# thangktran/HardwareAwareOptimalQuantumCircuitCuttingAndKnitting

Measured on AMD Instinct MI355X. Metric: subcircuit-instances/s (full-knit wall time = ms_per_step), syc 32 p=2, higher is better.
Workload: dtype f64

## Files before the change

### hardwareawareoptimalquantumcircuitcuttingandknitting_amd/_lib.py

```python
from __future__ import annotations

import ctypes
import os
import threading

_HERE = os.path.dirname(os.path.abspath(__file__))
LIB_PATH = os.environ.get("QKNIT_LIB") or os.path.join(_HERE, "libqknit.so")

c_i32, c_i64, c_u32, c_u64 = ctypes.c_int32, ctypes.c_int64, ctypes.c_uint32, ctypes.c_uint64
c_vp, c_dp, c_lp = ctypes.c_void_p, ctypes.POINTER(ctypes.c_double), ctypes.POINTER(ctypes.c_int64)


class QkPass(ctypes.Structure):
    _fields_ = [("tile_mask", c_u64), ("group_begin", c_i32), ("group_end", c_i32),
                ("flags", c_i32), ("traced_local", c_u32)]


class QkProgram(ctypes.Structure):
    _fields_ = [("n", c_i32), ("n_eff", c_i32), ("m", c_i32), ("n_slots", c_i32),
                ("packed", c_i32), ("n_passes", c_i32), ("passes", ctypes.POINTER(QkPass)),
                ("ops", c_vp), ("groups", c_vp), ("mats", c_vp)]


class QkLowrankPlan(ctypes.Structure):
# ... 54 lines not shown
    "qk_rank_factors": (c_i32, [c_vp, c_i64, c_vp, c_vp, ctypes.c_double, ctypes.c_double, ctypes.c_double,
                                ctypes.c_int, c_vp, c_vp, c_vp]),
    "qk_prep_workspace_bytes": (c_i32, [c_vp, c_i64, c_i64, ctypes.POINTER(c_i64)]),
    "qk_prep_operands": (c_i32, [c_vp, ctypes.c_int, ctypes.c_int, c_vp, c_vp, c_i64, c_i64, c_vp, ctypes.c_int,
                                 c_vp, c_vp, c_i64, c_i64, c_vp, c_vp, c_vp, c_vp, c_vp, c_vp, c_i64]),
    "qk_compress_operands": (c_i32, [c_vp, ctypes.c_int, ctypes.c_int, c_vp, c_vp, c_i64, c_vp, c_vp, c_vp, c_i64,
                                     c_vp]),
    "qk_compress_operands_ld": (c_i32, [c_vp, ctypes.c_int, ctypes.c_int, c_vp, c_vp, c_i64, c_i64, c_vp, c_i64, c_vp,
                                        c_vp, c_i64, c_i64, c_vp, c_i64]),
    "qk_compress_probe_v": (c_i32, [c_vp, ctypes.c_int, ctypes.c_int, c_vp, c_vp, c_i64, c_i64, c_vp, c_i64, c_vp, c_vp,
                                    c_i64, c_i64, c_vp, c_i64, c_vp, c_i64, c_vp, c_i64]),
    "qk_probe_errors_vpart": (c_i32, [c_vp, ctypes.c_int, ctypes.c_int, c_vp, c_i64, c_i64, c_vp, c_i64, c_vp, c_vp,
                                      c_i64, c_vp, c_vp, ctypes.c_double, ctypes.c_double, c_vp, c_vp, c_vp, c_i64,
                                      c_vp]),
    "qk_probe_workspace_bytes": (c_i32, [c_vp, c_i64, ctypes.POINTER(c_i64)]),
    "qk_probe_errors": (c_i32, [c_vp, ctypes.c_int, ctypes.c_int, c_vp, c_i64, c_i64, c_vp, c_i64, c_vp, c_vp, c_i64,
                                c_i64, c_vp, c_i64, c_vp, c_vp, ctypes.c_double, ctypes.c_double, c_vp, c_vp, c_vp,
                                c_i64]),
    "qk_probe_errors_tally": (c_i32, [c_vp, ctypes.c_int, ctypes.c_int, c_vp, c_i64, c_i64, c_vp, c_i64, c_vp, c_vp, c_i64,
                                c_i64, c_vp, c_i64, c_vp, c_vp, ctypes.c_double, ctypes.c_double, c_vp, c_vp, c_vp,
                                c_i64, c_vp]),
    "qk_probe_accept": (c_i32, [c_vp, c_vp, ctypes.c_int, c_vp, ctypes.c_double, ctypes.c_double, c_vp, c_vp]),
    "qk_rank_tally": (c_i32, [c_vp, c_vp, c_vp, c_vp]),
    "qk_knit_workspace_bytes": (c_i32, [ctypes.POINTER(QkKnitPlan), ctypes.POINTER(c_i64)]),
    "qk_knit": (c_i32, [c_vp, ctypes.POINTER(QkKnitPlan), c_vp, c_vp, c_i64, c_vp]),
    "qk_khatri_rao": (c_i32, [c_vp, c_i64, c_i64, c_i64, c_vp, c_i64, c_vp, c_i64, c_vp]),
    "qk_gather_rows": (c_i32, [c_vp, c_i64, c_i64, c_vp, c_vp, c_vp, c_vp]),
    "qk_npd_workspace_bytes": (c_i32, [c_i64, c_i64, ctypes.POINTER(c_i64)]),
    "qk_threshold_count": (c_i32, [c_vp, c_i64, c_vp, ctypes.c_double, c_vp, c_i64, c_vp]),
    "qk_npd": (c_i32, [c_vp, c_i64, c_vp, ctypes.c_double, c_i64, c_vp, c_i64, c_vp, c_vp, c_vp]),
    "qk_qd_from_rows": (c_i32, [c_vp, c_i64, c_i64, c_vp, c_vp, ctypes.c_double, c_vp]),
    "qk_qd_merge": (c_i32, [c_vp, c_i64, c_vp, c_vp, c_i64, c_vp, c_vp, ctypes.c_double, c_i64, c_vp]),
    "qk_qd_axpby": (c_i32, [c_vp, c_i64, ctypes.c_double, c_vp, ctypes.c_double, c_vp, ctypes.c_double, c_vp]),
    "qk_hellinger": (c_i32, [c_vp, c_i64, c_vp, c_vp, c_vp]),
    "qk_knit_lowrank_workspace_bytes": (c_i32, [c_vp, c_vp, ctypes.POINTER(c_i64)]),
    "qk_knit_lowrank": (c_i32, [c_vp, c_vp, c_vp, c_vp, c_vp, c_i64, c_vp, c_vp]),
    "qk_comm_unique_id": (c_i32, [c_vp]),
    "qk_comm_init": (c_i32, [c_vp, c_vp, ctypes.c_int, ctypes.c_int, ctypes.POINTER(c_vp)]),
    "qk_comm_destroy": (c_i32, [c_vp]),
    "qk_comm_size": (c_i32, [c_vp, ctypes.POINTER(ctypes.c_int), ctypes.POINTER(ctypes.c_int)]),
    "qk_allreduce": (c_i32, [c_vp, c_vp, c_vp, c_vp, c_i64]),
    "qk_reduce": (c_i32, [c_vp, c_vp, c_vp, c_vp, c_i64, ctypes.c_int]),
    "qk_allgather": (c_i32, [c_vp, c_vp, c_vp, c_vp, c_i64]),
    "qk_alltoall": (c_i32, [c_vp, c_vp, c_vp, c_vp, c_i64]),
    "qk_knit_select_workspace_bytes": (c_i32, [ctypes.c_int, c_u64, c_u64, ctypes.POINTER(c_i64)]),
    "qk_knit_select": (c_i32, [c_vp, ctypes.c_int, c_i64, c_vp, c_i64, c_vp, c_i64, c_u64, c_u64, ctypes.c_double,
# ... 58 lines not shown
```

### hardwareawareoptimalquantumcircuitcuttingandknitting_amd/csrc/internal.h

```cpp
#ifndef QKNIT_INTERNAL_H
#define QKNIT_INTERNAL_H

#include <hip/hip_runtime.h>

#include <string>

#include "../../include/qknit.h"

struct qk_ctx {
    int device;
    hipStream_t own;
    hipStream_t stream;
    int cus;
    std::string err;
};

size_t npd_pairs_bytes(int64_t count);
int npd_pairs_bits(qk_ctx* ctx, int64_t count, const int64_t* keys, const double* vals, int key_bits, void* ws,
                   int64_t ws_bytes, int64_t* out_keys, double* out_vals, int64_t* n_out_dev);

#endif
```

### hardwareawareoptimalquantumcircuitcuttingandknitting_amd/csrc/qknit.hip

```cpp
#include <hip/hip_runtime.h>

#include <cstdlib>

#include <cstdint>
#include <cstdio>
#include <cstring>
#include <string>

#include "internal.h"
#include "sweep_ops.h"

namespace {

constexpr int TILE = 1 << QK_TILE_BITS;
constexpr int NT = 256;

int fail(qk_ctx* ctx, int code, const char* fmt, const char* detail = "") {
    if (ctx) {
        char buf[512];
        snprintf(buf, sizeof(buf), fmt, detail);
        ctx->err = buf;
    }
    return code;
}
// ... 1348 lines not shown
static int stream_cus(hipStream_t s, int device) {
    int cus = 0;
    if (hipDeviceGetAttribute(&cus, hipDeviceAttributeMultiprocessorCount, device) != hipSuccess || cus < 1)
        cus = 1;
    uint32_t mask[32] = {0};
    if (s && hipExtStreamGetCUMask(s, 32, mask) == hipSuccess) {
        int n = 0;
        for (uint32_t w : mask) n += __builtin_popcount(w);
        if (n > 0 && n < cus) return n;
    }
    return cus;
}

int qk_ctx_create(int device, qk_ctx** out) {
    if (!out) return QK_EARG;
    *out = nullptr;
    if (hipSetDevice(device) != hipSuccess) return QK_EHIP;
    qk_ctx* c = new qk_ctx();
    c->device = device;
    if (hipStreamCreateWithFlags(&c->own, hipStreamNonBlocking) != hipSuccess) {
        delete c;
        return QK_EHIP;
    }
    c->stream = c->own;
    c->cus = stream_cus(c->own, device);
    *out = c;
    return QK_OK;
}

int qk_ctx_destroy(qk_ctx* ctx) {
    if (!ctx) return QK_EARG;
    (void)hipSetDevice(ctx->device);
    (void)hipStreamSynchronize(ctx->own);
    (void)hipStreamDestroy(ctx->own);
    delete ctx;
    return QK_OK;
}

int qk_ctx_set_stream(qk_ctx* ctx, void* s) {
    if (!ctx) return QK_EARG;
    if ((hipStream_t)s != ctx->stream || s == nullptr) ctx->cus = stream_cus((hipStream_t)s, ctx->device);
    ctx->stream = (hipStream_t)s;
    return QK_OK;
}

int qk_stream_create_cu_masked(int device, const uint32_t* cu_mask, int mask_words, void** stream) {
    if (!stream || !cu_mask || mask_words < 1 || mask_words > 32) return QK_EARG;
    *stream = nullptr;
    if (hipSetDevice(device) != hipSuccess) return QK_EHIP;
    int n = 0;
    for (int w = 0; w < mask_words; ++w) n += __builtin_popcount(cu_mask[w]);
    if (n == 0) return QK_EARG;
    hipStream_t s = nullptr;
    if (hipExtStreamCreateWithCUMask(&s, (uint32_t)mask_words, cu_mask) != hipSuccess) return QK_EHIP;
    *stream = s;
    return QK_OK;
// ... 321 lines not shown
```

### hardwareawareoptimalquantumcircuitcuttingandknitting_amd/csrc/qknit_plan.hip

```cpp
#include <hip/hip_runtime.h>

#include <algorithm>
#include <cstdlib>
#include <string>
#include <vector>

#include "internal.h"

namespace {

int pfail(qk_ctx* ctx, int code, const std::string& msg) {
    if (ctx) ctx->err = msg;
    return code;
}

__global__ void qk_pdep_keys_kernel(int64_t n, uint64_t mask, int64_t* keys) {
    for (int64_t x = blockIdx.x * (int64_t)blockDim.x + threadIdx.x; x < n; x += (int64_t)gridDim.x * blockDim.x) {
        uint64_t m = mask, k = 0, bit = 1;
        for (; m; m &= m - 1, bit <<= 1)
            if ((uint64_t)x & bit) k |= m & (~m + 1);
        keys[x] = (int64_t)k;
    }
}

// ... 242 lines not shown

int qk_knit_lowrank(qk_ctx* ctx, const qk_lowrank_plan* p, const double* q_a, const double* q_b, void* workspace,
                    int64_t workspace_bytes, double* out, int32_t* rank_out) {
    if (!ctx) return QK_EARG;
    LowrankLayout L;
    std::string why;
    int rc = lowrank_layout(ctx, p, L, why);
    if (rc) return pfail(ctx, rc, why);
    if (!q_a || !q_b || !out || !workspace || workspace_bytes < L.total)
        return pfail(ctx, QK_EARG, "qk_knit_lowrank: null rows / output, or workspace below qk_knit_lowrank_workspace_bytes");
    if (hipSetDevice(ctx->device) != hipSuccess) return pfail(ctx, QK_EHIP, "qk_knit_lowrank: hipSetDevice");
    char* ws = static_cast<char*>(workspace);
    auto D = [&](int64_t off) { return reinterpret_cast<double*>(ws + off); };
    const int K = p->terms;
    const int64_t NA = int64_t(1) << __builtin_popcountll(p->mask_a), NB = int64_t(1) << __builtin_popcountll(p->mask_b);
    double *XA = D(L.xa), *XB = D(L.xb), *G = D(L.g), *U = D(L.u);
    int32_t* r = reinterpret_cast<int32_t*>(ws + L.r);
    int32_t* k = reinterpret_cast<int32_t*>(ws + L.k);
    rc = qk_prep_operands(ctx, K, (int)p->rows_a, p->wt_a, q_a, NA, NA, XA, (int)p->rows_b, p->wt_b, q_b, NB, NB, XB,
                          p->probes, G, G + K * K, U, D(L.prep), L.prep_bytes);
    if (!rc) rc = qk_rank_factors(ctx, K, G, G + K * K, p->lam_tol, p->s_tol, p->s_abs, LR_RMAX, D(L.ta), D(L.tb), r);
    if (!rc) rc = qk_compress_operands(ctx, K, LR_RMAX, D(L.ta), XA, NA, D(L.a2), D(L.tb), XB, NB, D(L.b2));
    if (!rc)
        rc = qk_probe_errors(ctx, K, LR_RMAX, XA, NA, NA, D(L.a2), NA, U, D(L.b2), NB, NB, p->probes, NB, D(L.e2), r,
                             p->rank_tol, p->rank_tol_rel, k, D(L.err), D(L.probe), L.probe_bytes);
    if (!rc)
        rc = qk_knit_outer_stream_range(ctx, p->nbits, LR_RMAX, D(L.a2), NA, D(L.b2), NB, p->mask_a, p->mask_b, 0,
                                        int64_t(1) << p->nbits, k, out);
    if (rc) return rc;
    int64_t* ka = L.ka >= 0 ? reinterpret_cast<int64_t*>(ws + L.ka) : nullptr;
    int64_t* kb = L.kb >= 0 ? reinterpret_cast<int64_t*>(ws + L.kb) : nullptr;
    if (ka) hipLaunchKernelGGL(qk_pdep_keys_kernel, dim3(grid_of(NA)), dim3(256), 0, ctx->stream, NA, p->mask_a, ka);
    if (kb) hipLaunchKernelGGL(qk_pdep_keys_kernel, dim3(grid_of(NB)), dim3(256), 0, ctx->stream, NB, p->mask_b, kb);
    const int64_t sa = ka ? 0 : int64_t(1) << __builtin_ctzll(p->mask_a);
    const int64_t sb = kb ? 0 : int64_t(1) << __builtin_ctzll(p->mask_b);
    rc = qk_gemm_keyed_pred(ctx, NA, NB, K, XA, NA, XB, NB, ka, sa, kb, sb, out, 0, k);
    if (rc) return rc;
    if (rank_out) hipLaunchKernelGGL(qk_copy_i32_kernel, dim3(1), dim3(1), 0, ctx->stream, k, rank_out);
    if (hipGetLastError() != hipSuccess) return pfail(ctx, QK_EHIP, "qk_knit_lowrank: launch failed");
    return QK_OK;
}

}
```

### hardwareawareoptimalquantumcircuitcuttingandknitting_amd/csrc/qknit_prep.hip

```cpp
#include <hip/hip_runtime.h>

#include <cstdint>
#include <string>

#include "internal.h"

namespace {

typedef double d4_t __attribute__((ext_vector_type(4)));
typedef double d2_t __attribute__((ext_vector_type(2)));

constexpr int PK = 64;
constexpr int PCT = 128;
constexpr int PNP = 16;
constexpr int PTH = 512;
constexpr int XLD = PCT + 2;
constexpr int PG_BLK = 10;
constexpr int PPG = PG_BLK * 256;
constexpr int PPA = PPG;
constexpr int PPB = PPG + PK * PNP;
__host__ __device__ constexpr int prep_tri(int bi, int bj) { return bi * 4 - bi * (bi - 1) / 2 + (bj - bi); }

struct PrepSide {
    const double* Wt;
// ... 687 lines not shown
}

int fail(qk_ctx* ctx, int code, const char* msg) {
    ctx->err = msg;
    return code;
}

#ifndef QK_PREP_SPLIT
#define QK_PREP_SPLIT 1
#endif
bool prep_split(qk_ctx* ctx, int64_t NA, int64_t NB) {
    const int64_t tiles = (NA > NB ? NA : NB) / PCT;
    const int64_t g = (int64_t)(ctx->cus > 0 ? ctx->cus : 256) * QK_PREP_WG_PER_CU;
    return QK_PREP_SPLIT && tiles > 0 && 2 * tiles <= g;
}

int prep_grid(qk_ctx* ctx, int64_t NA, int64_t NB) {
    const int64_t tiles = (NA > NB ? NA : NB) / PCT;
    if (prep_split(ctx, NA, NB)) return (int)(2 * tiles);
    const int64_t g = (int64_t)(ctx->cus > 0 ? ctx->cus : 256) * QK_PREP_WG_PER_CU;
    return (int)(tiles < g ? (tiles > 0 ? tiles : 1) : g);
}

}

extern "C" {

int qk_prep_workspace_bytes(qk_ctx* ctx, int64_t NA, int64_t NB, int64_t* bytes) {
    if (!ctx || !bytes) return QK_EARG;
    *bytes = (int64_t)prep_grid(ctx, NA, NB) * (PPA + PPB) * (int64_t)sizeof(double);
    return QK_OK;
}

int qk_prep_operands(qk_ctx* ctx, int K, int RA, const double* WtA, const double* qA, int64_t ldqA, int64_t NA,
                     double* XA, int RB, const double* WtB, const double* qB, int64_t ldqB, int64_t NB, double* XB,
                     const double* probes, double* GA, double* GB, double* U, double* work, int64_t work_bytes) {
    if (!ctx) return QK_EARG;
    if (K < 2 || K > PK || (K & 1) || RA < 1 || RB < 1)
        return fail(ctx, QK_EARG, "qk_prep_operands: need even 2 <= K <= 64 and R >= 1 on both sides");
    if (((reinterpret_cast<uintptr_t>(WtA) | reinterpret_cast<uintptr_t>(WtB) | reinterpret_cast<uintptr_t>(qA) |
          reinterpret_cast<uintptr_t>(qB)) & 15) || (ldqA & 1) || (ldqB & 1))
        return fail(ctx, QK_EARG, "qk_prep_operands: 16-B aligned Wt / q and even ldq required");
    if (NA < PCT || NB < PCT || NA % PCT || NB % PCT || ldqA < NA || ldqB < NB)
        return fail(ctx, QK_EARG, "qk_prep_operands: columns must be a positive multiple of 128 (ldq >= N)");
    if (!WtA || !qA || !XA || !WtB || !qB || !XB || !probes || !GA || !GB || !U || !work)
        return fail(ctx, QK_EARG, "qk_prep_operands: null buffer");
// ... 102 lines not shown
    return QK_OK;
}

int qk_probe_workspace_bytes(qk_ctx* ctx, int64_t NA, int64_t* bytes) {
    if (!ctx || !bytes) return QK_EARG;
    *bytes = (int64_t)(PV_GRID * PV_PART + probe_grid_d(ctx, NA) * PE) * (int64_t)sizeof(double);
    return QK_OK;
}

int qk_probe_errors(qk_ctx* ctx, int K, int rmax, const double* XA, int64_t ldx, int64_t NA, const double* A2,
                    int64_t lda2, const double* U, const double* B2, int64_t ldb2, int64_t NB, const double* probes,
                    int64_t ldp, double* e2, const int32_t* r_dev, double tol, double rel_tol, int32_t* k_out,
                    double* err_out, double* work, int64_t work_bytes) {
    return qk_probe_errors_tally(ctx, K, rmax, XA, ldx, NA, A2, lda2, U, B2, ldb2, NB, probes, ldp, e2, r_dev, tol,
                                 rel_tol, k_out, err_out, work, work_bytes, nullptr);
}

int qk_probe_errors_tally(qk_ctx* ctx, int K, int rmax, const double* XA, int64_t ldx, int64_t NA, const double* A2,
                          int64_t lda2, const double* U, const double* B2, int64_t ldb2, int64_t NB,
                          const double* probes, int64_t ldp, double* e2, const int32_t* r_dev, double tol,
                          double rel_tol, int32_t* k_out, double* err_out, double* work, int64_t work_bytes,
                          int64_t* tally) {
    if (!ctx) return QK_EARG;
    if (K < 1 || K > PK || rmax < 1 || rmax > 8 || NA < 16 || NA % 16 || NB < 4 || NB % 4)
        return fail(ctx, QK_EARG, "qk_probe_errors: need 1 <= K <= 64, 1 <= rmax <= 8, NA % 16 == 0, NB % 4 == 0");
    if (!XA || !A2 || !U || !B2 || !probes || !work || (k_out && !r_dev) || (tally && !k_out))
        return fail(ctx, QK_EARG, "qk_probe_errors: null buffer");
    if (ldx < NA || ldb2 < NB || ldp < NB) return fail(ctx, QK_EARG, "qk_probe_errors: leading dimension");
    const int gd = probe_grid_d(ctx, NA);
    if (work_bytes < (int64_t)(PV_GRID * PV_PART + gd * PE) * (int64_t)sizeof(double))
        return fail(ctx, QK_EARG, "qk_probe_errors: workspace too small (qk_probe_workspace_bytes)");
    if (hipSetDevice(ctx->device) != hipSuccess) return fail(ctx, QK_EHIP, "qk_probe_errors: hipSetDevice");
    double* vpart = work;
    double* epart = work + PV_GRID * PV_PART;
    hipLaunchKernelGGL(qk_probe_v_kernel, dim3(PV_GRID), dim3(256), 0, ctx->stream, rmax, B2, ldb2, NB, probes, ldp,
                       vpart);
    hipLaunchKernelGGL(qk_probe_d_kernel, dim3(gd), dim3(256), 0, ctx->stream, K, rmax, XA, ldx, NA, A2, lda2, U, vpart,
                       PV_GRID, epart);
    hipLaunchKernelGGL(qk_probe_accept_kernel, dim3(1), dim3(256), 0, ctx->stream, epart, gd, r_dev, tol, rel_tol, e2,
                       k_out, err_out, tally);
    const hipError_t e = hipGetLastError();
    if (e != hipSuccess) return fail(ctx, QK_EHIP, (std::string("qk_probe_errors: ") + hipGetErrorString(e)).c_str());
    return QK_OK;
}

__global__ __launch_bounds__(64) void qk_rank_tally_kernel(const int32_t* __restrict__ r, const int32_t* __restrict__ k,
                                                          int64_t* __restrict__ acc) {
    if (threadIdx.x == 0) {
        const int rv = *r, kv = *k;
        acc[0] += rv == 0 ? 1 : 0;
        acc[1] += (rv > 0 && kv == 0) ? 1 : 0;
        acc[2] = kv;
        acc[3] += 1;
    }
}

int qk_rank_tally(qk_ctx* ctx, const int32_t* r_dev, const int32_t* k_dev, int64_t* acc) {
    if (!ctx) return QK_EARG;
    if (!r_dev || !k_dev || !acc) return fail(ctx, QK_EARG, "qk_rank_tally: null buffer");
    if (hipSetDevice(ctx->device) != hipSuccess) return fail(ctx, QK_EHIP, "qk_rank_tally: hipSetDevice");
    hipLaunchKernelGGL(qk_rank_tally_kernel, dim3(1), dim3(64), 0, ctx->stream, r_dev, k_dev, acc);
    const hipError_t e = hipGetLastError();
    if (e != hipSuccess) return fail(ctx, QK_EHIP, (std::string("qk_rank_tally: ") + hipGetErrorString(e)).c_str());
    return QK_OK;
}

// ... 14 lines not shown
```

### hardwareawareoptimalquantumcircuitcuttingandknitting_amd/engine.py

```python
from __future__ import annotations

import atexit
import contextlib
import ctypes
import dataclasses
import hashlib
import logging
import os
import threading
from dataclasses import dataclass, field
from time import perf_counter

import numpy as np

from . import _lib
from .fragment_program import (FragmentProgram, JobTable, basis_reduce, build_jobs, compile_fragment,
                               dedup_labels)
from .knit_plan import LabelSpace, deposit_keys, factor_vgate
from .sweep_plan import K_SLOT, EncodedProgram, encode

_torch = None


def torch():
# ... 1440 lines not shown
    ctx.check(ctx.lib.qk_probe_workspace_bytes(ctx.handle, NA, ctypes.byref(need)), "qk_probe_workspace_bytes")
    key = (str(dev), T.cuda.current_stream(dev).cuda_stream)
    work = _PROBE_WORK.get(key)
    if work is None or work.numel() * 8 < need.value:
        work = _PROBE_WORK[key] = T.empty(max(need.value // 8, 1), dtype=T.float64, device=dev)
    e2 = T.empty(2 * N_PROBES, dtype=T.float64, device=dev)
    k = T.empty(1, dtype=T.int32, device=dev) if r is not None else None
    err = T.empty(1, dtype=T.float64, device=dev) if r is not None else None
    assert tally is None or (r is not None and tally.dtype == T.int64 and tally.numel() == 4)
    if vpart is not None:
        assert vpart.is_contiguous() and vpart.shape[1:] == (8, N_PROBES)
        ctx.check(ctx.lib.qk_probe_errors_vpart(ctx.handle, K, rmax, XA.data_ptr(), XA.stride(0), NA,
                                                A2.data_ptr() + 8 * off, A2.shape[1], U.data_ptr(), vpart.data_ptr(),
                                                vpart.shape[0], e2.data_ptr(), _ptr(r), tol, rel_tol, _ptr(k), _ptr(err),
                                                work.data_ptr(), work.numel() * 8, _ptr(tally)), "qk_probe_errors_vpart")
        return e2, k, err
    ctx.check(ctx.lib.qk_probe_errors_tally(ctx.handle, K, rmax, XA.data_ptr(), XA.stride(0), NA, A2.data_ptr() + 8 * off,
                                            A2.shape[1], U.data_ptr(), B2.data_ptr(), NB, NB, probes.data_ptr(), NB,
                                            e2.data_ptr(), _ptr(r), tol, rel_tol, _ptr(k), _ptr(err), work.data_ptr(),
                                            work.numel() * 8, _ptr(tally)), "qk_probe_errors_tally")
    return e2, k, err


def probe_accept(ctx: Context, e2, r, tol: float, rel_tol: float = 0.0):
    T = torch()
    k = T.empty(1, dtype=T.int32, device=e2.device)
    err = T.empty(1, dtype=T.float64, device=e2.device)
    ctx.check(ctx.lib.qk_probe_accept(ctx.handle, e2.data_ptr(), 1, r.data_ptr(), tol, rel_tol, k.data_ptr(),
                                      err.data_ptr()), "qk_probe_accept")
    return k, err


def _endpoints(virt, j):
    out = [None, None]
    for instr in virt.circuit:
        op = instr.operation
        if getattr(op, "vgate_idx", None) == j:
            out[op.qubit_idx] = op
    return out


def factored_ok(virt) -> bool:
    frag_of = {}
    for frag in virt.fragment_circuits:
        for q in frag:
            frag_of[q] = frag
# ... 374 lines not shown
```

### hardwareawareoptimalquantumcircuitcuttingandknitting_amd/pipeline.py

```python
from __future__ import annotations

import ctypes
import os
import threading
from dataclasses import dataclass
from time import perf_counter

import numpy as np

from . import _lib, engine
from .fragment_program import JobTable


_PROBES: dict = {}
_PROBES_LOCK = threading.Lock()


def _mm_nt(X, Y):
    L = X.shape[1]
    nb = L // 256 if L % 256 == 0 else 1
    if nb <= 1:
        return X @ Y.T
    Xb = X.view(X.shape[0], nb, 256).transpose(0, 1)
    Yb = Y.reshape(Y.shape[0], nb, 256).transpose(0, 1)
# ... 121 lines not shown
    base = a._base
    if (base is not None and b._base is base and base.dim() == 1 and a.is_contiguous() and b.is_contiguous()
            and a.data_ptr() == base.data_ptr()
            and b.data_ptr() == a.data_ptr() + a.numel() * a.element_size()
            and base.numel() == a.numel() + b.numel()):
        return base
    return T.cat([a.reshape(-1), b.reshape(-1)])


class Backend:

    REQUIRED = ("prepare_fragments", "upload_jobs", "workspace_bytes", "empty", "zeros", "to_device", "sweep",
                "reduce_labels", "gather_rows", "gemm_keyed", "khatri_rao", "event")
    ROUTES = {
        "rank_factors": ("rank_factors", "compress", "probe_errors"),
        "prep_operands": ("prep_operands",),
        "sweep_rows": ("sweep_rows",),
        "plan_multi": ("plan_multi", "sweep_multi"),
        "knit_select": ("knit_select", "npd_pairs"),
        "out_buffer": ("out_buffer",),
        "knit_outer_stream": ("knit_outer_stream",),
        "gemm_outer_paired": ("gemm_outer_paired",),
    }
    OPTIONAL = ("sweep_labels", "fold_traced", "probe_accept", "select_above", "npd_dense")
    routes: frozenset = frozenset()
    dev = None
    fuses_tally = False
    shared_init = None

    def __init_subclass__(cls, **kw):
        super().__init_subclass__(**kw)
        needs = cls.REQUIRED + tuple(op for r in cls.routes for op in cls.ROUTES[r])
        known = (set(cls.REQUIRED) | set(cls.OPTIONAL) | {op for ops in cls.ROUTES.values() for op in ops}
                 | {n for n, v in vars(Backend).items() if callable(v)})
        bad = ([f"missing {n}" for n in needs if not callable(getattr(cls, n, None))]
               + [f"{n} is not a Backend operation" for n, v in vars(cls).items()
                  if callable(v) and not n.startswith("_") and n not in known])
        if bad:
            raise TypeError(f"{cls.__name__}: " + "; ".join(bad))

    @staticmethod
    def adopt(be):
        if not isinstance(be, Backend):
            kind = type(be)
            routes = frozenset(r for r, ops in Backend.ROUTES.items()
                               if all(callable(getattr(kind, op, None)) for op in ops))
            be.__class__ = type(kind.__name__, (kind, Backend), {"routes": routes})
        return be

    def device_width(self, fs) -> int:
        return 1 << fs.prog.m

    def fuses_labels(self, fs) -> bool:
        return False

    def bind(self):
        """Follow the caller's current stream (nothing to do on a host backend)."""

    def outer_stream_kernel(self, K, clbits_a, clbits_b, nbits, o_begin=0, o_count=None) -> str:
        return type(self).__name__

    def compress_v(self, TA, XA, TB, XB, probes, a_cols=None, a_width=None):
        return None

    def rank_tally(self, r, k, acc):
        T = engine.torch()
        rv, kv = int(r.reshape(-1)[0]), int(k.reshape(-1)[0])
        acc += T.tensor([int(rv == 0), int(rv > 0 and kv == 0), 0, 1], dtype=T.int64)
        acc[2] = kv


class HipBackend(Backend):

    routes = frozenset(Backend.ROUTES)

    def __init__(self, device: int = 0):
        self.T = engine.torch()
        self.device = device
        self.dev = self.T.device("cuda", device)
        self.ctx = engine.get_context(device)

    def prepare_fragments(self, virt, basis: bool = False, jit: bool | None = None, relevance: bool = True):
        return engine.prepare_fragments(virt, self.device, basis=basis, jit=jit, relevance=relevance)

    def upload_jobs(self, jobs: JobTable):
        return engine.jobs_to_device(jobs, self.device)
# ... 93 lines not shown
    def outer_stream_kernel(self, K, clbits_a, clbits_b, nbits, o_begin=0, o_count=None):
        return engine.knit_outer_stream_kernel(K, clbits_a, clbits_b, nbits, o_begin, o_count)

    def rank_factors(self, GA, GB):
        return engine.rank_factors_device(self.ctx, GA, GB)

    def prep_operands(self, WtA, qA, WtB, qB, probes):
        return engine.prep_operands(self.ctx, WtA, qA, WtB, qB, probes)

    fuses_tally = True

    def probe_errors(self, XA, A2, U, B2, probes, r=None, tol=0.0, a2_cols=None, rel_tol=0.0, tally=None, vpart=None):
        return engine.probe_errors(self.ctx, XA, A2, U, B2, probes, r=r, tol=tol, a2_cols=a2_cols, rel_tol=rel_tol,
                                   tally=tally, vpart=vpart)

    def compress_v(self, TA, XA, TB, XB, probes, a_cols=None, a_width=None):
        if os.environ.get("QKNIT_COMPRESS_V", "1") == "0" or not engine.compress_probe_v_ok(XA, XB, a_cols):
            return None
        return engine.compress_probe_v(self.ctx, TA, XA, TB, XB, probes, a_cols=a_cols, a_width=a_width)

    def probe_accept(self, e2, r, tol, rel_tol=0.0):
        return engine.probe_accept(self.ctx, e2, r, tol, rel_tol)

    def rank_tally(self, r, k, acc):
        self.ctx.check(self.ctx.lib.qk_rank_tally(self.ctx.handle, r.data_ptr(), k.data_ptr(), acc.data_ptr()),
                       "qk_rank_tally")

    def compress(self, TA, XA, TB, XB, a_cols=None, a_width=None):
        return engine.compress_operands(self.ctx, TA, XA, TB, XB, a_cols=a_cols, a_width=a_width)

    def knit_select(self, A, B, clbits_a, clbits_b, nbits, accuracy, k_dev=None):
        return engine.knit_select(self.ctx, A, B, clbits_a, clbits_b, nbits, accuracy, k_dev=k_dev)

    def npd_pairs(self, keys, vals):
        return engine.npd_pairs(self.ctx, keys, vals)

    def select_above(self, dense, accuracy, key_base=0):
        return engine.select_above(self.ctx, dense, accuracy, key_base=key_base)

    def npd_dense(self, dense, accuracy):
        return engine.nearest_probability_distribution(self.ctx, dense, accuracy)

    def out_buffer(self, n: int, select: bool = True):
        return engine.out_buffer(self.ctx, n, select=select)

    def event(self):
        return self.T.cuda.Event(enable_timing=True)


@dataclass
class PreparedStep:
    A2: object
    B2: object
    k_eff: object
    mats: list
    exact: object = None
    host_verdict: tuple | None = None
    exact_queued: bool = False


class KnitPipeline:
    def __init__(self, virt, device: int = 0, factored: bool = False, rank: int = 0, world: int = 1,
                 mode: str | None = None, group=None, backend=None, chunk_jobs: int | None = None,
                 jit: bool | None = None, light_cone: bool = True, data_rank: bool | None = None):
        self.be = Backend.adopt(backend) if backend is not None else HipBackend(device)
        self.chunk_jobs = int(os.environ.get("QKNIT_SWEEP_CHUNK_JOBS", "0")) if chunk_jobs is None else chunk_jobs
        self.fork = False
        self._multi = None
        self._streams = []
        self._sweep_graph = None
        self.T = engine.torch()
        self.virt = virt
        self.rank, self.world, self.group = rank, world, group
        factored = factored and engine.factored_ok(virt)
        self.factored = factored
        kw = {} if light_cone else {"relevance": False}
        if jit is not None:
            kw["jit"] = jit
        self.plan_ms = {}
        tick = perf_counter()
        with engine.host_planning():
# ... 426 lines not shown
                W = self.transforms[i]
                a = be.empty((W.shape[1], q.shape[1]), T.float64)
                be.gemm_keyed(W, q, out=a, strideA=q.shape[1])
            else:
                a = be.gather_rows(q, self.gather_idx[i], self.gather_coef[i])
            mats.append(a)
        return mats

    N_PROBES = 16
    RANK_GIVE_UP = 3

    def _probes(self, n: int, device):
        if self._probe is None or self._probe.shape[1] != n:
            key = (n, str(device))
            with _PROBES_LOCK:
                hit = _PROBES.get(key)
                if hit is None:
                    T = self.T
                    g = T.Generator().manual_seed(1234)
                    hit = _PROBES[key] = T.randn((self.N_PROBES, n), generator=g, dtype=T.float64).to(device)
            self._probe = hit
        return self._probe

    def _prep_step(self, qs) -> PreparedStep:
        return self._prep_slice(qs) if self.mode == "slice" and self.sharded else self._prep_dev_rank(qs)

    def _launch_step(self, p: PreparedStep):
        return self._launch_slice(p) if self.mode == "slice" else self._launch_dev_rank(p)

    def knit(self, qs: list):
        if self.dev_rank and self.mode in ("single", "slice"):
            p = self._prep_step(qs)
            if self.out is None:
                self.out = self._alloc_out(None)
            return self._launch_step(p)
        mats = self.operands(qs)
        if self.out is None:
            self.out = self._alloc_out(mats)
        if self.mode == "slice":
            ia, ib = self.order[0], self.order[-1]
            return self._slice_exact(mats[ia], mats[ib], self.ops.clbits[ia], self.ops.clbits[ib])
        low = self._rank_compress(mats) if self.data_rank else None
        if self.record_events:
            start, end = self.be.event(), self.be.event()
            start.record()
        if low is not None:
            res = self._contract_lowrank(low[0])
        elif self.mode == "single" and len(self.order) == 2 and mats[self.order[0]].shape[0] <= 8:
            res = self._contract_lowrank(mats)
        else:
            res = self._contract(mats)
        if self.record_events:
            end.record()
            self.events.append((start, end))
        if low is not None and not float(low[1]) <= max(self.rank_tol, self.rank_tol_rel * low[2]):
# ... 26 lines not shown
        qb = qs[ib] if qs[ib].stride(1) == 1 else qs[ib].contiguous()
        XA, XB, G, U = self.be.prep_operands(self.transforms[ia], qa, self.transforms[ib], qb, probes)
        mats = [None] * len(qs)
        mats[ia], mats[ib] = XA, XB
        self.last_prep = "fused"
        return mats, G, U

    def _accept(self, A, B, A2, B2, x, r, ref_rows=None, cmp_rows=None, reduce_err=None, note=True):
        T = self.T
        if ref_rows is None:
            ref_rows = A.T @ _mm_nt(B, x)
            cmp_rows = A2.T @ _mm_nt(B2, x)
        e2 = T.cat([((ref_rows - cmp_rows) ** 2).sum(dim=0), (ref_rows ** 2).sum(dim=0)])
        if reduce_err is not None:
            e2 = reduce_err(e2)
        n = e2.numel() // 2
        err = e2[:n].max().sqrt()
        bound = T.clamp(self.rank_tol_rel * e2[n:].max().sqrt(), min=self.rank_tol)
        k_eff = T.where((err <= bound) & (r > 0), r, T.zeros_like(r))
        if note:
            self._note_rank(r, k_eff)
        return k_eff, err

    def _prep_dev_rank(self, qs) -> PreparedStep:
        ia, ib = self.order[0], self.order[-1]
        if self._fused_prep(qs):
            x = self._probes(qs[ib].shape[1], qs[ib].device)
            mats, G, U = self._prep_fused(qs, x)
            TA, TB, r = self.be.rank_factors(G[0], G[1])
            return self._compress_and_check(TA, TB, r, mats, U, x)
        mats = self.operands(qs)
        self.last_prep = "torch"
        A, B = mats[ia], mats[ib]
        G = self.T.stack([_mm_nt(A, A), _mm_nt(B, B)])
        TA, TB, r = self.be.rank_factors(G[0].contiguous(), G[1].contiguous())
        A2, B2 = (TA @ A).contiguous(), (TB @ B).contiguous()
        k_eff, _ = self._accept(A, B, A2, B2, self._probes(B.shape[1], B.device), r)
        return PreparedStep(A2, B2, k_eff, mats)

    def _compress_and_check(self, TA, TB, r, mats, U, x) -> PreparedStep:
        ia, ib = self.order[0], self.order[-1]
        a_cols = self._replicated_a_cols()
        kw = {"a_cols": a_cols} if a_cols is not None else {}
        cv = self.be.compress_v(TA, mats[ia], TB, mats[ib], x, **kw)
        check = {}
        if cv is not None:
            A2, B2, check["vpart"] = cv
        else:
            A2, B2 = self.be.compress(TA, mats[ia], TB, mats[ib], **kw)
        XA = mats[ia]
        if a_cols is not None:
            XA = XA[:, a_cols[0]:a_cols[0] + a_cols[1]]
            check["a2_cols"] = a_cols
        tally = self.be.fuses_tally
        if tally:
            check["tally"] = self._tally_for(r.device)
        _, k_eff, _ = self.be.probe_errors(XA, A2, U, B2, x, r=r, tol=self.rank_tol, rel_tol=self.rank_tol_rel,
                                           **check)
        if tally:
            self._pending += 1
        else:
            self._note_rank(r, k_eff)
        return PreparedStep(A2, B2, k_eff, mats)

    def _launch_dev_rank(self, p: PreparedStep):
        ia, ib = self.order[0], self.order[-1]
        cA, cB = self.ops.clbits[ia], self.ops.clbits[ib]
        if self.record_events:
            start, end = self.be.event(), self.be.event()
            start.record()
        self.last_kernel = self.be.outer_stream_kernel(p.A2.shape[0], cA, cB, self.N)
        self.be.knit_outer_stream(p.A2, p.B2, cA, cB, self.N, self.out, k_dev=p.k_eff)
        if self.record_events:
            end.record()
            self.events.append((start, end))
        return self._contract(p.mats, skip=p.k_eff)

    def _broadcast_factors(self, TA, TB, r):
        import torch.distributed as dist

        T = self.T
        R8, K = TA.shape
        fac = T.cat([TA.reshape(-1), TB.reshape(-1), r.to(T.float64)])
        dist.broadcast(fac, src=self._group_rank0(), group=self.group)
        return fac[:R8 * K].view(R8, K), fac[R8 * K:2 * R8 * K].view(R8, K), fac[-1:].to(T.int32)

    def _prep_slice(self, qs) -> PreparedStep:
        import torch.distributed as dist

        T, be, P = self.T, self.be, self.world
        ia, ib = self.order[0], self.order[-1]
        bwA, bwB = qs[ia].shape[1], qs[ib].shape[1]
        x_full = self._probes(bwB * P, qs[ib].device)
        if self._x_local is None or self._x_local.shape[1] != bwB:
            self._x_local = x_full[:, self.rank * bwB:(self.rank + 1) * bwB].contiguous()
# ... 661 lines not shown
```

### include/qknit.h

```cpp
#ifndef QKNIT_H
#define QKNIT_H

#include <stdint.h>

#ifdef __cplusplus
extern "C" {
#endif

#define QK_OK 0
#define QK_EARG 1
#define QK_EHIP 2
#define QK_ESTATE 3

#define QK_TILE_BITS 12
#define QK_FIBER_BITS 4

enum { QK_U1 = 0, QK_D1 = 1, QK_SLOT = 2, QK_U2 = 3, QK_D2 = 4, QK_CX = 5, QK_SWAP = 6, QK_SCALE = 7,
       QK_U1R = 8, QK_U1X = 9, QK_D1R = 10, QK_D2R = 11, QK_SCALER = 12 };

typedef struct qk_op {
    int32_t kind;
    int32_t a, b;
    int32_t e1, e2;
    int32_t slot;
// ... 169 lines not shown
int qk_compress_probe_v(qk_ctx* ctx, int K, int rmax, const double* TA, const double* XA, int64_t NA, int64_t ldxa,
                        double* A2, int64_t lda2, const double* TB, const double* XB, int64_t NB, int64_t ldxb,
                        double* B2, int64_t ldb2, const double* probes, int64_t ldp, double* vpart,
                        int64_t vpart_doubles);

int qk_probe_errors_vpart(qk_ctx* ctx, int K, int rmax, const double* XA, int64_t ldx, int64_t NA, const double* A2,
                          int64_t lda2, const double* U, const double* vpart, int64_t gv, double* e2,
                          const int32_t* r_dev, double tol, double rel_tol, int32_t* k_out, double* err_out,
                          double* work, int64_t work_bytes, int64_t* tally);

int qk_probe_workspace_bytes(qk_ctx* ctx, int64_t NA, int64_t* bytes);
int qk_probe_errors(qk_ctx* ctx, int K, int rmax, const double* XA, int64_t ldx, int64_t NA, const double* A2,
                    int64_t lda2, const double* U, const double* B2, int64_t ldb2, int64_t NB, const double* probes,
                    int64_t ldp, double* e2, const int32_t* r_dev, double tol, double rel_tol, int32_t* k_out,
                    double* err_out, double* work, int64_t work_bytes);
int qk_probe_errors_tally(qk_ctx* ctx, int K, int rmax, const double* XA, int64_t ldx, int64_t NA, const double* A2,
                          int64_t lda2, const double* U, const double* B2, int64_t ldb2, int64_t NB,
                          const double* probes, int64_t ldp, double* e2, const int32_t* r_dev, double tol,
                          double rel_tol, int32_t* k_out, double* err_out, double* work, int64_t work_bytes,
                          int64_t* tally);
int qk_probe_accept(qk_ctx* ctx, const double* e2, int n, const int32_t* r_dev, double tol, double rel_tol,
                    int32_t* k_out, double* err_out);
int qk_rank_tally(qk_ctx* ctx, const int32_t* r_dev, const int32_t* k_dev, int64_t* acc);


int qk_npd_workspace_bytes(int64_t n, int64_t count, int64_t* bytes);

int qk_threshold_count(qk_ctx* ctx, int64_t n, const double* vals, double acc, void* ws, int64_t ws_bytes,
                       int64_t* count_dev);

int qk_npd(qk_ctx* ctx, int64_t n, const double* vals, double acc, int64_t count, void* ws, int64_t ws_bytes,
           int64_t* out_keys, double* out_vals, int64_t* n_out_dev);

int qk_select_above(qk_ctx* ctx, int64_t n, const double* vals, double acc, int64_t key_base, int64_t capacity,
                    int64_t* keys, double* out_vals, int64_t* count_dev);


int qk_sample_cdf(qk_ctx* ctx, int64_t n_seg, const int64_t* seg_off, int64_t width, const double* pjob,
                  double* cdf);

int qk_sample_counts(qk_ctx* ctx, int64_t n_labels, int64_t label_base, const int64_t* label_seg,
                     const int64_t* seg_off, const int64_t* label_row_off, int64_t width, const double* cdf,
                     int64_t shots, uint64_t seed, unsigned int* counts);

int qk_fold_counts(qk_ctx* ctx, int64_t n_labels, const int64_t* label_row_off, int64_t width,
                   const double* row_sign, const unsigned int* counts, int64_t shots, double acc, double* q);
// ... 81 lines not shown
```

Baseline: 523,000.

## Add checked outer knit that can overlap rank probe with speculative write

Adds a fused qk_knit_outer_checked entry point that runs the probe/accept kernels and then the outer-product stream write. When QKNIT_SPEC_WRITE is enabled, the probe runs on a side stream and the write runs concurrently, using the proposed rank r instead of the accepted k. A join event makes the main stream wait for the probe. The plain single-mode knit path now routes through this function, which also skips the separate compress_v step. The speculative mode is off by default, so the default path runs probe then write on one stream. The speculative write uses r, which may differ from the accepted rank k.

```diff
diff --git a/hardwareawareoptimalquantumcircuitcuttingandknitting_amd/_lib.py b/hardwareawareoptimalquantumcircuitcuttingandknitting_amd/_lib.py
--- a/hardwareawareoptimalquantumcircuitcuttingandknitting_amd/_lib.py
+++ b/hardwareawareoptimalquantumcircuitcuttingandknitting_amd/_lib.py
@@ -100,6 +100,10 @@
                                 c_i64, c_vp]),
     "qk_probe_accept": (c_i32, [c_vp, c_vp, ctypes.c_int, c_vp, ctypes.c_double, ctypes.c_double, c_vp, c_vp]),
     "qk_rank_tally": (c_i32, [c_vp, c_vp, c_vp, c_vp]),
+    "qk_knit_outer_checked_mode": (c_i32, [c_vp, ctypes.POINTER(ctypes.c_int)]),
+    "qk_knit_outer_checked": (c_i32, [c_vp, ctypes.c_int, ctypes.c_int, c_vp, c_i64, c_i64, c_vp, c_i64, c_vp, c_vp, c_i64,
+                                      c_i64, c_vp, c_i64, c_vp, c_vp, ctypes.c_double, ctypes.c_double, c_vp, c_vp, c_vp,
+                                      c_i64, c_vp, ctypes.c_int, c_u64, c_u64, c_i64, c_i64, c_vp]),
     "qk_knit_workspace_bytes": (c_i32, [ctypes.POINTER(QkKnitPlan), ctypes.POINTER(c_i64)]),
     "qk_knit": (c_i32, [c_vp, ctypes.POINTER(QkKnitPlan), c_vp, c_vp, c_i64, c_vp]),
     "qk_khatri_rao": (c_i32, [c_vp, c_i64, c_i64, c_i64, c_vp, c_i64, c_vp, c_i64, c_vp]),
diff --git a/hardwareawareoptimalquantumcircuitcuttingandknitting_amd/csrc/internal.h b/hardwareawareoptimalquantumcircuitcuttingandknitting_amd/csrc/internal.h
--- a/hardwareawareoptimalquantumcircuitcuttingandknitting_amd/csrc/internal.h
+++ b/hardwareawareoptimalquantumcircuitcuttingandknitting_amd/csrc/internal.h
@@ -13,6 +13,8 @@
     hipStream_t stream;
     int cus;
     std::string err;
+    hipStream_t side;
+    hipEvent_t fork, join;
 };
 
 size_t npd_pairs_bytes(int64_t count);
diff --git a/hardwareawareoptimalquantumcircuitcuttingandknitting_amd/csrc/qknit.hip b/hardwareawareoptimalquantumcircuitcuttingandknitting_amd/csrc/qknit.hip
--- a/hardwareawareoptimalquantumcircuitcuttingandknitting_amd/csrc/qknit.hip
+++ b/hardwareawareoptimalquantumcircuitcuttingandknitting_amd/csrc/qknit.hip
@@ -1394,6 +1394,18 @@
         delete c;
         return QK_EHIP;
     }
+    c->side = nullptr;
+    c->fork = c->join = nullptr;
+    if (hipStreamCreateWithFlags(&c->side, hipStreamNonBlocking) != hipSuccess ||
+        hipEventCreateWithFlags(&c->fork, hipEventDisableTiming) != hipSuccess ||
+        hipEventCreateWithFlags(&c->join, hipEventDisableTiming) != hipSuccess) {
+        if (c->join) (void)hipEventDestroy(c->join);
+        if (c->fork) (void)hipEventDestroy(c->fork);
+        if (c->side) (void)hipStreamDestroy(c->side);
+        (void)hipStreamDestroy(c->own);
+        delete c;
+        return QK_EHIP;
+    }
     c->stream = c->own;
     c->cus = stream_cus(c->own, device);
     *out = c;
@@ -1403,7 +1415,11 @@
 int qk_ctx_destroy(qk_ctx* ctx) {
     if (!ctx) return QK_EARG;
     (void)hipSetDevice(ctx->device);
+    (void)hipStreamSynchronize(ctx->side);
     (void)hipStreamSynchronize(ctx->own);
+    (void)hipEventDestroy(ctx->join);
+    (void)hipEventDestroy(ctx->fork);
+    (void)hipStreamDestroy(ctx->side);
     (void)hipStreamDestroy(ctx->own);
     delete ctx;
     return QK_OK;
diff --git a/hardwareawareoptimalquantumcircuitcuttingandknitting_amd/csrc/qknit_plan.hip b/hardwareawareoptimalquantumcircuitcuttingandknitting_amd/csrc/qknit_plan.hip
--- a/hardwareawareoptimalquantumcircuitcuttingandknitting_amd/csrc/qknit_plan.hip
+++ b/hardwareawareoptimalquantumcircuitcuttingandknitting_amd/csrc/qknit_plan.hip
@@ -288,11 +288,9 @@
     if (!rc) rc = qk_rank_factors(ctx, K, G, G + K * K, p->lam_tol, p->s_tol, p->s_abs, LR_RMAX, D(L.ta), D(L.tb), r);
     if (!rc) rc = qk_compress_operands(ctx, K, LR_RMAX, D(L.ta), XA, NA, D(L.a2), D(L.tb), XB, NB, D(L.b2));
     if (!rc)
-        rc = qk_probe_errors(ctx, K, LR_RMAX, XA, NA, NA, D(L.a2), NA, U, D(L.b2), NB, NB, p->probes, NB, D(L.e2), r,
-                             p->rank_tol, p->rank_tol_rel, k, D(L.err), D(L.probe), L.probe_bytes);
-    if (!rc)
-        rc = qk_knit_outer_stream_range(ctx, p->nbits, LR_RMAX, D(L.a2), NA, D(L.b2), NB, p->mask_a, p->mask_b, 0,
-                                        int64_t(1) << p->nbits, k, out);
+        rc = qk_knit_outer_checked(ctx, K, LR_RMAX, XA, NA, NA, D(L.a2), NA, U, D(L.b2), NB, NB, p->probes, NB, D(L.e2),
+                                   r, p->rank_tol, p->rank_tol_rel, k, D(L.err), D(L.probe), L.probe_bytes, nullptr,
+                                   p->nbits, p->mask_a, p->mask_b, 0, int64_t(1) << p->nbits, out);
     if (rc) return rc;
     int64_t* ka = L.ka >= 0 ? reinterpret_cast<int64_t*>(ws + L.ka) : nullptr;
     int64_t* kb = L.kb >= 0 ? reinterpret_cast<int64_t*>(ws + L.kb) : nullptr;
diff --git a/hardwareawareoptimalquantumcircuitcuttingandknitting_amd/csrc/qknit_prep.hip b/hardwareawareoptimalquantumcircuitcuttingandknitting_amd/csrc/qknit_prep.hip
--- a/hardwareawareoptimalquantumcircuitcuttingandknitting_amd/csrc/qknit_prep.hip
+++ b/hardwareawareoptimalquantumcircuitcuttingandknitting_amd/csrc/qknit_prep.hip
@@ -733,6 +733,37 @@
     return (int)(tiles < g ? (tiles > 0 ? tiles : 1) : g);
 }
 
+int probe_check_args(qk_ctx* ctx, int K, int rmax, const double* XA, int64_t ldx, int64_t NA, const double* A2,
+                     const double* U, const double* B2, int64_t ldb2, int64_t NB, const double* probes, int64_t ldp,
+                     const int32_t* r_dev, const int32_t* k_out, const double* work, int64_t work_bytes,
+                     const int64_t* tally) {
+    if (K < 1 || K > PK || rmax < 1 || rmax > 8 || NA < 16 || NA % 16 || NB < 4 || NB % 4)
+        return fail(ctx, QK_EARG, "qk_probe_errors: need 1 <= K <= 64, 1 <= rmax <= 8, NA % 16 == 0, NB % 4 == 0");
+    if (!XA || !A2 || !U || !B2 || !probes || !work || (k_out && !r_dev) || (tally && !k_out))
+        return fail(ctx, QK_EARG, "qk_probe_errors: null buffer");
+    if (ldx < NA || ldb2 < NB || ldp < NB) return fail(ctx, QK_EARG, "qk_probe_errors: leading dimension");
+    if (work_bytes < (int64_t)(PV_GRID * PV_PART + probe_grid_d(ctx, NA) * PE) * (int64_t)sizeof(double))
+        return fail(ctx, QK_EARG, "qk_probe_errors: workspace too small (qk_probe_workspace_bytes)");
+    return QK_OK;
+}
+
+int probe_check_on(qk_ctx* ctx, hipStream_t s, int K, int rmax, const double* XA, int64_t ldx, int64_t NA,
+                   const double* A2, int64_t lda2, const double* U, const double* B2, int64_t ldb2, int64_t NB,
+                   const double* probes, int64_t ldp, double* e2, const int32_t* r_dev, double tol, double rel_tol,
+                   int32_t* k_out, double* err_out, double* work, int64_t* tally) {
+    const int gd = probe_grid_d(ctx, NA);
+    double* vpart = work;
+    double* epart = work + PV_GRID * PV_PART;
+    hipLaunchKernelGGL(qk_probe_v_kernel, dim3(PV_GRID), dim3(256), 0, s, rmax, B2, ldb2, NB, probes, ldp, vpart);
+    hipLaunchKernelGGL(qk_probe_d_kernel, dim3(gd), dim3(256), 0, s, K, rmax, XA, ldx, NA, A2, lda2, U, vpart, PV_GRID,
+                       epart);
+    hipLaunchKernelGGL(qk_probe_accept_kernel, dim3(1), dim3(256), 0, s, epart, gd, r_dev, tol, rel_tol, e2, k_out,
+                       err_out, tally);
+    const hipError_t e = hipGetLastError();
+    if (e != hipSuccess) return fail(ctx, QK_EHIP, (std::string("qk_probe_errors: ") + hipGetErrorString(e)).c_str());
+    return QK_OK;
+}
+
 }
 
 extern "C" {
@@ -881,26 +912,77 @@
                           double rel_tol, int32_t* k_out, double* err_out, double* work, int64_t work_bytes,
                           int64_t* tally) {
     if (!ctx) return QK_EARG;
-    if (K < 1 || K > PK || rmax < 1 || rmax > 8 || NA < 16 || NA % 16 || NB < 4 || NB % 4)
-        return fail(ctx, QK_EARG, "qk_probe_errors: need 1 <= K <= 64, 1 <= rmax <= 8, NA % 16 == 0, NB % 4 == 0");
-    if (!XA || !A2 || !U || !B2 || !probes || !work || (k_out && !r_dev) || (tally && !k_out))
-        return fail(ctx, QK_EARG, "qk_probe_errors: null buffer");
-    if (ldx < NA || ldb2 < NB || ldp < NB) return fail(ctx, QK_EARG, "qk_probe_errors: leading dimension");
-    const int gd = probe_grid_d(ctx, NA);
-    if (work_bytes < (int64_t)(PV_GRID * PV_PART + gd * PE) * (int64_t)sizeof(double))
-        return fail(ctx, QK_EARG, "qk_probe_errors: workspace too small (qk_probe_workspace_bytes)");
+    const int rc = probe_check_args(ctx, K, rmax, XA, ldx, NA, A2, U, B2, ldb2, NB, probes, ldp, r_dev, k_out, work,
+                                    work_bytes, tally);
+    if (rc) return rc;
     if (hipSetDevice(ctx->device) != hipSuccess) return fail(ctx, QK_EHIP, "qk_probe_errors: hipSetDevice");
-    double* vpart = work;
-    double* epart = work + PV_GRID * PV_PART;
-    hipLaunchKernelGGL(qk_probe_v_kernel, dim3(PV_GRID), dim3(256), 0, ctx->stream, rmax, B2, ldb2, NB, probes, ldp,
-                       vpart);
-    hipLaunchKernelGGL(qk_probe_d_kernel, dim3(gd), dim3(256), 0, ctx->stream, K, rmax, XA, ldx, NA, A2, lda2, U, vpart,
-                       PV_GRID, epart);
-    hipLaunchKernelGGL(qk_probe_accept_kernel, dim3(1), dim3(256), 0, ctx->stream, epart, gd, r_dev, tol, rel_tol, e2,
-                       k_out, err_out, tally);
-    const hipError_t e = hipGetLastError();
-    if (e != hipSuccess) return fail(ctx, QK_EHIP, (std::string("qk_probe_errors: ") + hipGetErrorString(e)).c_str());
+    return probe_check_on(ctx, ctx->stream, K, rmax, XA, ldx, NA, A2, lda2, U, B2, ldb2, NB, probes, ldp, e2, r_dev, tol,
+                          rel_tol, k_out, err_out, work, tally);
+}
+
+constexpr bool SPEC_WRITE_DEFAULT = false;
+
+int qk_knit_outer_checked_mode(qk_ctx* ctx, int* speculative) {
+    if (!ctx || !speculative) return QK_EARG;
+    *speculative = 0;
+    const char* env = getenv("QKNIT_SPEC_WRITE");
+    if (!(env ? atoi(env) != 0 : SPEC_WRITE_DEFAULT)) return QK_OK;
+    if (hipSetDevice(ctx->device) != hipSuccess) return fail(ctx, QK_EHIP, "qk_knit_outer_checked: hipSetDevice");
+    int dev_cus = 0;
+    hipStreamCaptureStatus cap = hipStreamCaptureStatusNone;
+    if (hipDeviceGetAttribute(&dev_cus, hipDeviceAttributeMultiprocessorCount, ctx->device) != hipSuccess ||
+        hipStreamIsCapturing(ctx->stream, &cap) != hipSuccess)
+        return fail(ctx, QK_EHIP, "qk_knit_outer_checked: device / stream query");
+    *speculative = ctx->cus >= dev_cus && cap == hipStreamCaptureStatusNone;
     return QK_OK;
+}
+
+int qk_knit_outer_checked(qk_ctx* ctx, int K, int rmax, const double* XA, int64_t ldx, int64_t NA, const double* A2,
+                          int64_t lda2, const double* U, const double* B2, int64_t ldb2, int64_t NB,
+                          const double* probes, int64_t ldp, double* e2, const int32_t* r_dev, double tol,
+                          double rel_tol, int32_t* k_out, double* err_out, double* work, int64_t work_bytes,
+                          int64_t* tally, int nbits, uint64_t maskA, uint64_t maskB, int64_t o_begin, int64_t o_count,
+                          double* out) {
+    if (!ctx) return QK_EARG;
+    if (!r_dev || !k_out || !out) return fail(ctx, QK_EARG, "qk_knit_outer_checked: null r_dev / k_out / out");
+    int rc = probe_check_args(ctx, K, rmax, XA, ldx, NA, A2, U, B2, ldb2, NB, probes, ldp, r_dev, k_out, work,
+                              work_bytes, tally);
+    if (rc) return rc;
+    if (nbits < 2 || nbits > 32 || lda2 < NA || NA != int64_t(1) << __builtin_popcountll(maskA) ||
+        NB != int64_t(1) << __builtin_popcountll(maskB))
+        return fail(ctx, QK_EARG, "qk_knit_outer_checked: need 2 <= nbits <= 32, NA = 2^|maskA|, NB = 2^|maskB|");
+    if ((maskA & maskB) || (maskA | maskB) != (uint64_t(1) << nbits) - 1 || !(maskB & 1))
+        return fail(ctx, QK_EARG, "qk_knit_outer_checked: masks must be disjoint, cover all bits, bit 0 in B");
+    int kind = 0, tb = 0;
+    if (o_begin < 0 || o_count < 1 || o_begin + o_count > (int64_t(1) << nbits) ||
+        qk_knit_outer_stream_kind(nbits, rmax, maskA, maskB, o_begin, o_count, &kind, &tb) != QK_OK)
+        return fail(ctx, QK_EARG, "qk_knit_outer_checked: output range outside 0..2^nbits");
+    if (kind == 0 && (o_begin != 0 || o_count != (int64_t(1) << nbits)))
+        return fail(ctx, QK_EARG, "qk_knit_outer_checked: output ranges need task-aligned ranges of >= 2^9");
+    if (hipSetDevice(ctx->device) != hipSuccess) return fail(ctx, QK_EHIP, "qk_knit_outer_checked: hipSetDevice");
+    int spec = 0;
+    if (kind != 0 && (rc = qk_knit_outer_checked_mode(ctx, &spec)) != QK_OK) return rc;
+    if (!spec) {
+        rc = probe_check_on(ctx, ctx->stream, K, rmax, XA, ldx, NA, A2, lda2, U, B2, ldb2, NB, probes, ldp, e2, r_dev,
+                            tol, rel_tol, k_out, err_out, work, tally);
+        if (rc) return rc;
+        return qk_knit_outer_stream_range(ctx, nbits, rmax, A2, lda2, B2, ldb2, maskA, maskB, o_begin, o_count,
+                                          kind != 0 ? k_out : nullptr, out);
+    }
+    if (hipEventRecord(ctx->fork, ctx->stream) != hipSuccess || hipStreamWaitEvent(ctx->side, ctx->fork, 0) != hipSuccess)
+        return fail(ctx, QK_EHIP, "qk_knit_outer_checked: fork");
+    rc = probe_check_on(ctx, ctx->side, K, rmax, XA, ldx, NA, A2, lda2, U, B2, ldb2, NB, probes, ldp, e2, r_dev, tol,
+                        rel_tol, k_out, err_out, work, tally);
+    const bool joined = hipEventRecord(ctx->join, ctx->side) == hipSuccess;
+    int wrc = QK_OK;
+    if (!rc)
+        wrc = qk_knit_outer_stream_range(ctx, nbits, rmax, A2, lda2, B2, ldb2, maskA, maskB, o_begin, o_count, r_dev,
+                                         out);
+    if (!joined || hipStreamWaitEvent(ctx->stream, ctx->join, 0) != hipSuccess) {
+        (void)hipStreamSynchronize(ctx->side);
+        if (!rc && !wrc) return fail(ctx, QK_EHIP, "qk_knit_outer_checked: join");
+    }
+    return rc ? rc : wrc;
 }
 
 __global__ __launch_bounds__(64) void qk_rank_tally_kernel(const int32_t* __restrict__ r, const int32_t* __restrict__ k,
diff --git a/hardwareawareoptimalquantumcircuitcuttingandknitting_amd/engine.py b/hardwareawareoptimalquantumcircuitcuttingandknitting_amd/engine.py
--- a/hardwareawareoptimalquantumcircuitcuttingandknitting_amd/engine.py
+++ b/hardwareawareoptimalquantumcircuitcuttingandknitting_amd/engine.py
@@ -1486,6 +1486,41 @@
     return e2, k, err
 
 
+def checked_write_speculates(ctx: Context) -> bool:
+    spec = ctypes.c_int()
+    ctx.check(ctx.lib.qk_knit_outer_checked_mode(ctx.handle, ctypes.byref(spec)), "qk_knit_outer_checked_mode")
+    return bool(spec.value)
+
+
+def knit_outer_checked(ctx: Context, XA, A2, U, B2, probes, r, clbits_a: list, clbits_b: list, nbits: int, out,
+                       tol: float = 0.0, rel_tol: float = 0.0, tally=None):
+    T = torch()
+    K, NA = XA.shape
+    rmax, NB = B2.shape
+    assert A2.shape == (rmax, NA) and U.shape == (K, N_PROBES) and probes.shape == (N_PROBES, NB) and 1 <= rmax <= 8
+    assert all(t.is_contiguous() for t in (XA, A2, U, B2, probes))
+    assert NA == 1 << len(clbits_a) and NB == 1 << len(clbits_b) and out.numel() >= 1 << nbits
+    assert r.dtype == T.int32 and r.device == out.device
+    assert tally is None or (tally.dtype == T.int64 and tally.numel() == 4)
+    mA, mB = sum(1 << c for c in clbits_a), sum(1 << c for c in clbits_b)
+    dev = XA.device
+    need = ctypes.c_int64()
+    ctx.check(ctx.lib.qk_probe_workspace_bytes(ctx.handle, NA, ctypes.byref(need)), "qk_probe_workspace_bytes")
+    key = (str(dev), T.cuda.current_stream(dev).cuda_stream)
+    work = _PROBE_WORK.get(key)
+    if work is None or work.numel() * 8 < need.value:
+        work = _PROBE_WORK[key] = T.empty(max(need.value // 8, 1), dtype=T.float64, device=dev)
+    e2 = T.empty(2 * N_PROBES, dtype=T.float64, device=dev)
+    k = T.empty(1, dtype=T.int32, device=dev)
+    err = T.empty(1, dtype=T.float64, device=dev)
+    ctx.check(ctx.lib.qk_knit_outer_checked(ctx.handle, K, rmax, XA.data_ptr(), NA, NA, A2.data_ptr(), NA, U.data_ptr(),
+                                            B2.data_ptr(), NB, NB, probes.data_ptr(), NB, e2.data_ptr(), r.data_ptr(),
+                                            tol, rel_tol, k.data_ptr(), err.data_ptr(), work.data_ptr(),
+                                            work.numel() * 8, _ptr(tally), nbits, mA, mB, 0, 1 << nbits,
+                                            out.data_ptr()), "qk_knit_outer_checked")
+    return e2, k, err
+
+
 def probe_accept(ctx: Context, e2, r, tol: float, rel_tol: float = 0.0):
     T = torch()
     k = T.empty(1, dtype=T.int32, device=e2.device)
diff --git a/hardwareawareoptimalquantumcircuitcuttingandknitting_amd/pipeline.py b/hardwareawareoptimalquantumcircuitcuttingandknitting_amd/pipeline.py
--- a/hardwareawareoptimalquantumcircuitcuttingandknitting_amd/pipeline.py
+++ b/hardwareawareoptimalquantumcircuitcuttingandknitting_amd/pipeline.py
@@ -167,7 +167,7 @@
         "knit_outer_stream": ("knit_outer_stream",),
         "gemm_outer_paired": ("gemm_outer_paired",),
     }
-    OPTIONAL = ("sweep_labels", "fold_traced", "probe_accept", "select_above", "npd_dense")
+    OPTIONAL = ("sweep_labels", "fold_traced", "probe_accept", "select_above", "npd_dense", "knit_outer_checked")
     routes: frozenset = frozenset()
     dev = None
     fuses_tally = False
@@ -207,6 +207,9 @@
 
     def compress_v(self, TA, XA, TB, XB, probes, a_cols=None, a_width=None):
         return None
+
+    def checked_write(self) -> bool:
+        return False
 
     def rank_tally(self, r, k, acc):
         T = engine.torch()
@@ -346,6 +349,14 @@
     def probe_accept(self, e2, r, tol, rel_tol=0.0):
         return engine.probe_accept(self.ctx, e2, r, tol, rel_tol)
 
+    def checked_write(self) -> bool:
+        return engine.checked_write_speculates(self.ctx)
+
+    def knit_outer_checked(self, XA, A2, U, B2, probes, r, clbits_a, clbits_b, nbits, out, tol=0.0, rel_tol=0.0,
+                           tally=None):
+        return engine.knit_outer_checked(self.ctx, XA, A2, U, B2, probes, r, clbits_a, clbits_b, nbits, out, tol=tol,
+                                         rel_tol=rel_tol, tally=tally)
+
     def rank_tally(self, r, k, acc):
         self.ctx.check(self.ctx.lib.qk_rank_tally(self.ctx.handle, r.data_ptr(), k.data_ptr(), acc.data_ptr()),
                        "qk_rank_tally")
@@ -381,6 +392,7 @@
     exact: object = None
     host_verdict: tuple | None = None
     exact_queued: bool = False
+    check: tuple | None = None
 
 
 class KnitPipeline:
@@ -853,15 +865,17 @@
             self._probe = hit
         return self._probe
 
-    def _prep_step(self, qs) -> PreparedStep:
-        return self._prep_slice(qs) if self.mode == "slice" and self.sharded else self._prep_dev_rank(qs)
+    def _prep_step(self, qs, plain: bool = False) -> PreparedStep:
+        if self.mode == "slice" and self.sharded:
+            return self._prep_slice(qs)
+        return self._prep_dev_rank(qs, checked_write=plain and self.mode == "single")
 
     def _launch_step(self, p: PreparedStep):
         return self._launch_slice(p) if self.mode == "slice" else self._launch_dev_rank(p)
 
     def knit(self, qs: list):
         if self.dev_rank and self.mode in ("single", "slice"):
-            p = self._prep_step(qs)
+            p = self._prep_step(qs, plain=True)
             if self.out is None:
                 self.out = self._alloc_out(None)
             return self._launch_step(p)
@@ -934,13 +948,13 @@
             self._note_rank(r, k_eff)
         return k_eff, err
 
-    def _prep_dev_rank(self, qs) -> PreparedStep:
+    def _prep_dev_rank(self, qs, checked_write: bool = False) -> PreparedStep:
         ia, ib = self.order[0], self.order[-1]
         if self._fused_prep(qs):
             x = self._probes(qs[ib].shape[1], qs[ib].device)
             mats, G, U = self._prep_fused(qs, x)
             TA, TB, r = self.be.rank_factors(G[0], G[1])
-            return self._compress_and_check(TA, TB, r, mats, U, x)
+            return self._compress_and_check(TA, TB, r, mats, U, x, checked_write)
         mats = self.operands(qs)
         self.last_prep = "torch"
         A, B = mats[ia], mats[ib]
@@ -950,10 +964,14 @@
         k_eff, _ = self._accept(A, B, A2, B2, self._probes(B.shape[1], B.device), r)
         return PreparedStep(A2, B2, k_eff, mats)
 
-    def _compress_and_check(self, TA, TB, r, mats, U, x) -> PreparedStep:
+    def _compress_and_check(self, TA, TB, r, mats, U, x, checked_write: bool = False) -> PreparedStep:
         ia, ib = self.order[0], self.order[-1]
         a_cols = self._replicated_a_cols()
         kw = {"a_cols": a_cols} if a_cols is not None else {}
+        if checked_write and a_cols is None and self.be.checked_write():
+            A2, B2 = self.be.compress(TA, mats[ia], TB, mats[ib])
+            tally = self._tally_for(r.device) if self.be.fuses_tally else None
+            return PreparedStep(A2, B2, None, mats, check=(U, x, r, tally))
         cv = self.be.compress_v(TA, mats[ia], TB, mats[ib], x, **kw)
         check = {}
         if cv is not None:
@@ -982,7 +1000,17 @@
             start, end = self.be.event(), self.be.event()
             start.record()
         self.last_kernel = self.be.outer_stream_kernel(p.A2.shape[0], cA, cB, self.N)
-        self.be.knit_outer_stream(p.A2, p.B2, cA, cB, self.N, self.out, k_dev=p.k_eff)
+        if p.check is not None:
+            U, x, r, tally = p.check
+            _, p.k_eff, _ = self.be.knit_outer_checked(p.mats[ia], p.A2, U, p.B2, x, r, cA, cB, self.N, self.out,
+                                                       tol=self.rank_tol, rel_tol=self.rank_tol_rel, tally=tally)
+            p.check = None
+            if tally is not None:
+                self._pending += 1
+            else:
+                self._note_rank(r, p.k_eff)
+        else:
+            self.be.knit_outer_stream(p.A2, p.B2, cA, cB, self.N, self.out, k_dev=p.k_eff)
         if self.record_events:
             end.record()
             self.events.append((start, end))
diff --git a/include/qknit.h b/include/qknit.h
--- a/include/qknit.h
+++ b/include/qknit.h
@@ -215,6 +215,14 @@
 int qk_probe_accept(qk_ctx* ctx, const double* e2, int n, const int32_t* r_dev, double tol, double rel_tol,
                     int32_t* k_out, double* err_out);
 int qk_rank_tally(qk_ctx* ctx, const int32_t* r_dev, const int32_t* k_dev, int64_t* acc);
+
+int qk_knit_outer_checked_mode(qk_ctx* ctx, int* speculative);
+int qk_knit_outer_checked(qk_ctx* ctx, int K, int rmax, const double* XA, int64_t ldx, int64_t NA, const double* A2,
+                          int64_t lda2, const double* U, const double* B2, int64_t ldb2, int64_t NB,
+                          const double* probes, int64_t ldp, double* e2, const int32_t* r_dev, double tol,
+                          double rel_tol, int32_t* k_out, double* err_out, double* work, int64_t work_bytes,
+                          int64_t* tally, int nbits, uint64_t maskA, uint64_t maskB, int64_t o_begin, int64_t o_count,
+                          double* out);
 
 
 int qk_npd_workspace_bytes(int64_t n, int64_t count, int64_t* bytes);
```

Result: no change. 523,100, median of 3 (+0.0%).
